# rasmusbarr/nudge

Hardware: AMD Instinct MI355X
Metric: simulation steps/s (contacts solved/s alongside), 1M-box drop scene (higher is better)
Workload: dtype f32

## Files before the change

### nudge_amd/csrc/nh_solve.hip

```cpp
#include "nh_internal.h"
int nh_asleep_remember(nh_context* ctx);
#include <type_traits>
#include <atomic>
#include <string.h>
#include "nh_solver.h"
#include "nh_narrowphase.h"

#define NH_NONE 0xFFFFFFFFu
#define NH_CLS_NONE 0u
#define NH_CLS_STATIC4 1u
#define NH_CLS_STATIC8 2u
#define NH_CLS_STATICN 3u
#define NH_CLS_GENERAL 4u
#define NH_CLS_PENDING 0xFFu
#define NH_CLS_STATIC4_LATE 5u
#define NH_CLS_STATIC8_LATE 6u
#define NH_UNSET 0xFFFFFFFFu

__device__ __forceinline__ bool tag_less(uint64_t ta, uint32_t fa, uint64_t tb, uint32_t fb) { return ta < tb || (ta == tb && fa < fb); }

__global__ __launch_bounds__(256) void k_gravity(const nh_DevState* __restrict__ st, const uint32_t* __restrict__ active, nh_BodyMomentum* __restrict__ momentum,
                                                 float gx_dt, float gy_dt, float gz_dt, float damping) {
	uint32_t n = st->active;
	for (uint32_t k = blockIdx.x * blockDim.x + threadIdx.x; k < n; k += gridDim.x * blockDim.x) {
// ... 858 lines not shown
		uint32_t nf[M], of[M];
		uint32_t sl[M], jm[M];
#pragma unroll
		for (int k = 0; k < M; ++k) { nf[k] = 0u; of[k] = 0u; sl[k] = (uint32_t)k; jm[k] = 0xFFFFFFFFu; }
		if (STILL) {
			still_has = br != NH_BODY_REC_NONE;
			still_rec = still_has ? (br & ~NH_BODY_REC_IS_A) : 0u;
			const uint32_t n_bb = min(cv.st->pairs, sv.pair_cap);
			still_base = still_rec < n_bb ? 4u * still_rec : 4u * n_bb + (still_rec - n_bb);
			const uint32_t bp = still_has ? bpos : 0u;
			st_cnt = sv.cnt_sorted[bp]; st_start = sv.start_sorted[bp]; st_oc = sv.sc_count[still_rec];
			if (PAIR) {
				const uint2 kp = still_rec < n_bb ? av.kept[still_rec] : av.kept[av.kept_cap - 1u - (still_rec - n_bb)];
				const uint64_t pk = av.rec_key[still_rec];
				s_pk[wave][0][lane] = kp.x; s_pk[wave][1][lane] = kp.y; s_pk[wave][2][lane] = (uint32_t)pk; s_pk[wave][3][lane] = (uint32_t)(pk >> 32);
			}
#pragma unroll
			for (int k = 0; k < M; ++k) { nf[k] = sv.raw_feature[still_base + k]; of[k] = sv.sc_feat[still_base + k]; }
			s_first[wave][lane] = still_has ? still_base : 0xFFFFFFFFu;
		} else {
		if (CONTIG) cnt = sp.y & 15u;
		else if (mine) { b = off[x]; cnt = off[x + 1] - b; }
#pragma unroll
		for (int q = 0; q < M; ++q) {
			if (CONTIG) cid[q] = (uint32_t)q < cnt ? sp.x + ((sp.y >> (4 + 3 * q)) & 7u) : 0xFFFFFFFFu;
			else cid[q] = (uint32_t)q < cnt ? adj[b + q] : 0xFFFFFFFFu;
			first = min(first, cid[q]);
		}
		}
		if (!STILL) {
#pragma unroll
			for (int q = 0; q < M; ++q) scid[lane * M + q] = cid[q];
			s_hint[wave][lane] = h; s_first[wave][lane] = first;
		}
		const bool ghost_lane = AHEAD && fs.ghost_first != 0u && x >= fs.ghost_first;
		if (AHEAD) { if (!mine || ghost_lane) col = 0xFFFFFFFFu; s_col[wave][lane] = col; }
		__builtin_amdgcn_wave_barrier();
		uint32_t sc[M], sflags[M];
		float4 sc0[M], sc1[M], sw[M];
		uint64_t stag[M], sctag[M];
		uint32_t sfeat[M], scfeat[M], sguess[M];
#pragma unroll
		for (int k = 0; k < M; ++k) {
			const uint32_t e = 64u * k + lane, j = e / M;
			if (STILL) { const uint32_t bj = s_first[wave][j]; sc[k] = bj != 0xFFFFFFFFu ? bj + (e - j * M) : 0xFFFFFFFFu; }
			else sc[k] = scid[e];
			const uint32_t c = sc[k] != 0xFFFFFFFFu ? sc[k] : 0u;
			sc0[k] = reinterpret_cast<const float4*>(contacts + c)[0];
			sc1[k] = reinterpret_cast<const float4*>(contacts + c)[1];
			sflags[k] = (!CONTIG && bodies[c].a == wave_x0 + j) ? 2u : 0u;
			if (STILL) {
				sw[k] = *reinterpret_cast<const float4*>(cv.cdata + c);
			} else if (FUSED) {
				const uint32_t hj = s_hint[wave][j];
				sguess[k] = hj != NH_HINT_NONE ? hj + (sc[k] - s_first[wave][j]) : sc[k];
				const uint32_t g = sguess[k] < m ? sguess[k] : 0u;
				stag[k] = cv.tags[c]; sfeat[k] = cv.features[c];
				sctag[k] = cv.ctags[g]; scfeat[k] = cv.cfeatures[g];
				sw[k] = *reinterpret_cast<const float4*>(cv.cdata + g);
			} else {
				sw[k] = states[c];
			}
		}
		float4 m0 = make_float4(0, 0, 0, 0), m1 = m0, pr = m0, t0 = m0, t1 = make_float4(0, 0, 0, 1);
		uint32_t idle_early = 0;
		if (mine) {
			m0 = reinterpret_cast<const float4*>(momentum + x)[0]; m1 = reinterpret_cast<const float4*>(momentum + x)[1];
			pr = *reinterpret_cast<const float4*>(props + x);
			t0 = reinterpret_cast<const float4*>(xf + x)[0]; t1 = reinterpret_cast<const float4*>(xf + x)[1];
			if (CONTIG && (fs.bits & 2u)) idle_early = (STILL && (fs.bits & 4u)) ? idle0 : fs.idle[x];
			if (CONTIG && (fs.bits & 1u)) {
				float vel[3] = { m0.x, m0.y, m0.z }, ang[3] = { m1.x, m1.y, m1.z };
				nh_gravity_damping(vel, ang, fs.gx_dt, fs.gy_dt, fs.gz_dt, fs.damping);
				m0.x = vel[0]; m0.y = vel[1]; m0.z = vel[2]; m1.x = ang[0]; m1.y = ang[1]; m1.z = ang[2];
			}
		}
#pragma unroll
		for (int k = 0; k < M; ++k) {
			const uint32_t e = 64u * k + lane;
			nh_ob_slot o;
			o.c0 = make_float4(0, 0, 0, 0); o.c1 = o.c0; o.w = o.c0;
			if (sc[k] != 0xFFFFFFFFu) {
				uint32_t flags = sflags[k];
				o.c0 = sc0[k]; o.c1 = sc1[k];
				if (STILL) {
					o.w = make_float4(sw[k].x, sw[k].y, sw[k].z, __uint_as_float(flags));
				} else if (FUSED) {
					const bool hit = sguess[k] < m && sctag[k] == stag[k] && scfeat[k] == sfeat[k];
					if (!hit) flags |= 1u;
					o.w = hit ? make_float4(sw[k].x, sw[k].y, sw[k].z, __uint_as_float(flags)) : make_float4(0.0f, 0.0f, 0.0f, __uint_as_float(flags));
				} else {
					o.w = make_float4(sw[k].x, sw[k].y, sw[k].z, __uint_as_float(flags));
				}
			}
			slot[e] = o;
		}
		if (STILL) {
			uint32_t oc = 0;
			if (still_has) {
				cnt = min(st_cnt, 4u); oc = min(st_oc, 4u);
				uint32_t start = st_start;
				int shift = 0;
				for (uint32_t k = 0; k < n_delta; ++k) shift += (uint32_t)s_delta[k].x < bpos ? s_delta[k].y : 0;
				if (shift) { start += (uint32_t)shift; sv.start_sorted[bpos] = start; }
				st_start = start;
			}
			uint32_t ci[M], key[M];
#pragma unroll
			for (int k = 0; k < M; ++k) {
				uint32_t r = 0;
#pragma unroll
				for (int j = 0; j < M; ++j) r += ((uint32_t)j < cnt && (uint32_t)k < cnt && (nf[j] < nf[k] || (nf[j] == nf[k] && j < k))) ? 1u : 0u;
				const bool on = (uint32_t)k < cnt;
				ci[k] = on ? st_start + r : 0xFFFFFFFFu;
				key[k] = on ? slot_key_of(ci[k], nullptr) : 0xFFFFFFFFu;
				sl[k] = (uint32_t)k;
			}
#pragma unroll
			for (int q = 1; q < M; ++q) {
#pragma unroll
				for (int j = q; j > 0; --j) {
					const bool sw2 = (key[j] < key[j - 1]) || (key[j] == key[j - 1] && ci[j] < ci[j - 1]);
					const uint32_t tc = sw2 ? ci[j - 1] : ci[j], tk = sw2 ? key[j - 1] : key[j], ts = sw2 ? sl[j - 1] : sl[j];
					ci[j - 1] = sw2 ? ci[j] : ci[j - 1]; key[j - 1] = sw2 ? key[j] : key[j - 1]; sl[j - 1] = sw2 ? sl[j] : sl[j - 1];
					ci[j] = tc; key[j] = tk; sl[j] = ts;
				}
			}
#pragma unroll
			for (int q = 0; q < M; ++q) {
				const bool on = (uint32_t)q < cnt;
				uint32_t f = 0, wj = 0xFFFFFFFFu;
#pragma unroll
				for (int k = 0; k < M; ++k) if (sl[q] == (uint32_t)k) f = nf[k];
#pragma unroll
				for (int j = M - 1; j >= 0; --j) if ((uint32_t)j < oc && of[j] == f) wj = (uint32_t)j;
				jm[q] = on ? wj : 0xFFFFFFFFu;
				cid[q] = on ? still_base + sl[q] : 0xFFFFFFFFu;
				scid[lane * M + q] = cid[q];
			}
			if (still_has) {
#pragma unroll
				for (int k = 0; k < M; ++k) if ((uint32_t)k < cnt) sv.sc_feat[still_base + k] = nf[k];
				sv.sc_count[still_rec] = cnt;
			}
		}
		__builtin_amdgcn_wave_barrier();
		nh_vel v = { m0.x, m0.y, m0.z, pr.w, m1.x, m1.y, m1.z, m1.w };
		const nh_quat qx = { t1.x, t1.y, t1.z, t1.w };
		const nh_inertia IX = nh_world_inertia(qx, pr.x, pr.y, pr.z);
		const nh_f3 posx = nh_make3(t0.x, t0.y, t0.z);
		nh_row1 r[M];
		nh_state s[M];
		bool is_a[M];
#pragma unroll
		for (int q = 0; q < M; ++q) {
			is_a[q] = false;
			if ((uint32_t)q < cnt) {
				const nh_ob_slot o = slot[lane * M + (STILL ? sl[q] : (uint32_t)q)];
				const uint32_t flags = STILL ? 0u : __float_as_uint(o.w.w);
				is_a[q] = STILL ? (br & NH_BODY_REC_IS_A) != 0 : (CONTIG ? ((sp.y >> 28) & 1u) != 0 : (flags & 2u) != 0);
				nh_contact_in ci = { o.c0.x, o.c0.y, o.c0.z, o.c0.w, o.c1.x, o.c1.y, o.c1.z, o.c1.w };
				nh_build_row1(ci, posx, IX, v.mass_inverse, is_a[q], r[q]);
				if (FUSED) {
					float wx = o.w.x, wy = o.w.y, wz = o.w.z;
					if (STILL) {
						const float4 wv = slot[lane * M + (jm[q] != 0xFFFFFFFFu ? jm[q] : 0u)].w;
						const bool hit = jm[q] != 0xFFFFFFFFu;
						wx = hit ? wv.x : 0.0f; wy = hit ? wv.y : 0.0f; wz = hit ? wv.z : 0.0f;
					}
					if (!STILL && (flags & 1u)) {
						const float4 found = cache_search(cv.ctags, cv.cfeatures, cv.cdata, m, h != NH_HINT_NONE ? h + (cid[q] - first) : cid[q], cv.tags[cid[q]], cv.features[cid[q]]);
						wx = found.x; wy = found.y; wz = found.z;
					}
					nh_warm_start1(r[q], wx, wy, wz, v, is_a[q], s[q]);
				} else {
					s[q].normal = o.w.x; s[q].friction_x = o.w.y; s[q].friction_y = o.w.z;
				}
			}
		}
		if (FUSED && !STILL && mine) hint[x] = first;
		nh_xform pp_x = nh_xform();
		float4 pp_min = make_float4(0, 0, 0, 0), pp_max = pp_min, pp_shape = pp_min;
		uint32_t pp_tag = 0, pp_own_tag = 0, pp_partner = 0xFFFFFFFFu, pp_bits = 0;
		if (PAIR && CONTIG && (fs.bits & 2u) && mine && still_has && s_col[wave][lane] != 0xFFFFFFFFu) {
			const uint32_t ah_col = s_col[wave][lane];
			const uint32_t kx = s_pk[wave][0][lane], ky = s_pk[wave][1][lane];
			const uint32_t index_mask = av.gen ? NH_GEN_INDEX : 0xFFFFFFFFu;
			const uint32_t ca = kx & index_mask, cb = ky & index_mask;
			pp_partner = ca == ah_col ? cb : ca;
			pp_bits = 1u | ((ca != ah_col && cb != ah_col) ? 4u : 0u);
			if (av.gen && cv.st->moved_count != 0u && !((uint32_t)(av.gen[ca] & 0x7Fu) == (kx >> NH_GEN_SHIFT) && (uint32_t)(av.gen[cb] & 0x7Fu) == (ky >> NH_GEN_SHIFT))) pp_bits |= 2u;
			pp_x = av.xf[pp_partner]; pp_min = av.aabb_min[pp_partner]; pp_max = av.aabb_max[pp_partner];
			if (pp_partner < av.nbox) pp_shape = *reinterpret_cast<const float4*>(av.box_data + pp_partner);
			else pp_shape.x = av.sph_data[pp_partner - av.nbox].radius;
			pp_tag = av.ctag[pp_partner]; pp_own_tag = av.ctag[ah_col];
		}
		float4* const s_ah = reinterpret_cast<float4*>(slot);
		float ah_rad = 0.0f;
		if (AHEAD) {
			__builtin_amdgcn_wave_barrier();
			const uint32_t c0 = s_col[wave][lane];
			const uint32_t cc = c0 != 0xFFFFFFFFu ? c0 : 0u;
			const bool is_box = cc < av.nbox;
			const float4* lp = reinterpret_cast<const float4*>(is_box ? av.box_xf + cc : av.sph_xf + (cc - av.nbox));
			const float4* sp4 = is_box ? reinterpret_cast<const float4*>(av.box_data + cc) : lp;
			if (!is_box) ah_rad = av.sph_data[cc - av.nbox].radius;
			nh_glds16(lp, &s_ah[lane]); nh_glds16(lp + 1, &s_ah[64u + lane]);
			nh_glds16(av.fat_box + 2u * (size_t)cc, &s_ah[128u + lane]); nh_glds16(av.fat_box + 2u * (size_t)cc + 1u, &s_ah[192u + lane]);
			nh_glds16(sp4, &s_ah[256u + lane]);
		}
		if (CONTIG && __builtin_amdgcn_ballot_w64(mine && (STILL ? (still_has && (br & NH_BODY_REC_IS_A) != 0) : ((sp.y >> 28) & 1u) != 0)) == 0) {
			for (uint32_t it = 0; it < iterations; ++it) {
#pragma unroll
				for (int q = 0; q < M; ++q)
					if ((uint32_t)q < cnt) nh_apply_one1(r[q], s[q], v, false);
			}
		} else {
			for (uint32_t it = 0; it < iterations; ++it) {
#pragma unroll
				for (int q = 0; q < M; ++q)
					if ((uint32_t)q < cnt) nh_apply_one1(r[q], s[q], v, is_a[q]);
			}
		}
		float4 a0 = make_float4(0, 0, 0, 0), a1 = a0;
		uint32_t idle_in = 0;
		const bool advance_here = CONTIG && (fs.bits & 2u) && mine;
		float4 ah_l0 = make_float4(0, 0, 0, 0), ah_l1 = ah_l0, ah_fmn = ah_l0, ah_fmx = ah_l0, ah_sz = ah_l0;
		uint32_t ah_col = 0xFFFFFFFFu;
		if (AHEAD) {
			ah_col = s_col[wave][lane];
			asm volatile("s_waitcnt vmcnt(0)" ::: "memory");
			ah_l0 = s_ah[lane]; ah_l1 = s_ah[64u + lane]; ah_fmn = s_ah[128u + lane]; ah_fmx = s_ah[192u + lane]; ah_sz = s_ah[256u + lane];
		}
		if (advance_here) { a0 = t0; a1 = t1; idle_in = idle_early; }
		__builtin_amdgcn_wave_barrier();
#pragma unroll
		for (int q = 0; q < M; ++q) {
			if ((uint32_t)q < cnt) {
				float ox, oy, oz;
				nh_export_impulse1(r[q], s[q], ox, oy, oz);
				slot[lane * M + q].c0 = make_float4(s[q].normal, s[q].friction_x, s[q].friction_y, 0.0f);
				slot[lane * M + q].c1 = make_float4(ox, oy, oz, 0.0f);
			}
		}
		__builtin_amdgcn_wave_barrier();
#pragma unroll
		for (int k = 0; k < M; ++k) {
			const uint32_t e = 64u * k + lane;
			const uint32_t c = scid[e];
			if (c != 0xFFFFFFFFu) {
				if (keep_states) states[c] = slot[e].c0;
				*reinterpret_cast<float4*>(out_impulses + c) = slot[e].c1;
			}
		}
		if (mine) {
			reinterpret_cast<float4*>(momentum + x)[0] = make_float4(v.vx, v.vy, v.vz, v.mass_inverse);
			reinterpret_cast<float4*>(momentum + x)[1] = make_float4(v.wx, v.wy, v.wz, v.w_unused);
		}
		uint32_t nmin[3] = { 0xffffffffu, 0xffffffffu, 0xffffffffu }, nmax[3] = { 0u, 0u, 0u }, ntop = 0u;
		bool nfail = false;
		int pp_count = 0;
		float pair_scale = 0.0f;
		if (PAIR) {
			__builtin_amdgcn_wave_barrier();
#pragma unroll
			for (int k = 0; k < M; ++k) scid[lane * M + k] = 0xFFFFFFFFu;
			const nh_DevState* const sp = cv.st;
			const nh_f3 smin = nh_make3(nh_float_unflip(sp->still_smin[sv.parity][0]), nh_float_unflip(sp->still_smin[sv.parity][1]), nh_float_unflip(sp->still_smin[sv.parity][2]));
			const nh_f3 smax = nh_make3(nh_float_unflip(sp->still_smax[sv.parity][0]), nh_float_unflip(sp->still_smax[sv.parity][1]), nh_float_unflip(sp->still_smax[sv.parity][2]));
			pair_scale = nh_morton_scale(smin, smax);
			if (sp->pair_unowned > av.unowned_cap) nfail = true;
		}
		if (advance_here) {
			float pos[3] = { a0.x, a0.y, a0.z }, rot[4] = { a1.x, a1.y, a1.z, a1.w };
			const float vel[3] = { v.vx, v.vy, v.vz }, ang[3] = { v.wx, v.wy, v.wz };
			const uint8_t idle_out = nh_advance_body(pos, rot, vel, ang, (uint8_t)idle_in, fs.time_step);
			fs.idle[x] = idle_out;
			reinterpret_cast<float4*>(xf + x)[0] = make_float4(pos[0], pos[1], pos[2], a0.w);
			reinterpret_cast<float4*>(xf + x)[1] = make_float4(rot[0], rot[1], rot[2], rot[3]);
			if (AHEAD && !ghost_lane) {
				ntop = idle_out; nfail = idle_out == 0xffu;
				const uint32_t c = ah_col;
				if (c != 0xFFFFFFFFu) {
					const bool is_box = c < av.nbox;
					const float4 l0 = ah_l0, l1 = ah_l1, fmn = ah_fmn, fmx = ah_fmx;
					float4 sz = ah_sz;
					if (!is_box) sz.x = ah_rad;
					const nh_quat bq = { rot[0], rot[1], rot[2], rot[3] };
					const nh_quat lq = { l1.x, l1.y, l1.z, l1.w };
					const nh_f3 p = nh_rotate(bq, nh_make3(l0.x, l0.y, l0.z)) + nh_make3(pos[0], pos[1], pos[2]);
					const nh_quat q = nh_qmul(bq, lq);
					float sx, sy, sz2;
					if (is_box) {
						const nh_m33 m = nh_matrix(q);
						const nh_f3 c0 = m.c0 * sz.x, c1 = m.c1 * sz.y, c2 = m.c2 * sz.z;
						sx = fabsf(c0.x) + fabsf(c1.x) + fabsf(c2.x);
						sy = fabsf(c0.y) + fabsf(c1.y) + fabsf(c2.y);
						sz2 = fabsf(c0.z) + fabsf(c1.z) + fabsf(c2.z);
					} else {
						sx = sy = sz2 = sz.x;
					}
					const float mnx = p.x - sx, mny = p.y - sy, mnz = p.z - sz2, mxx = p.x + sx, mxy = p.y + sy, mxz = p.z + sz2;
					float4* const wx = reinterpret_cast<float4*>(av.xf) + 2u * (size_t)c;
					wx[0] = make_float4(p.x, p.y, p.z, l0.w);
					wx[1] = make_float4(q.x, q.y, q.z, q.s);
					av.aabb_min[c] = make_float4(mnx, mny, mnz, l0.w);
					av.aabb_max[c] = make_float4(mxx, mxy, mxz, __uint_as_float(0u));
					nfail |= !(mnx >= fmn.x && mny >= fmn.y && mnz >= fmn.z && mxx <= fmx.x && mxy <= fmx.y && mxz <= fmx.z);
					nmin[0] = nmax[0] = nh_float_flip(mnx); nmin[1] = nmax[1] = nh_float_flip(mny); nmin[2] = nmax[2] = nh_float_flip(mnz);
					if (PAIR && (pp_bits & 1u)) {
						const float4 omin = make_float4(mnx, mny, mnz, l0.w), omax = make_float4(mxx, mxy, mxz, 0.0f);
						nh_xform OX; OX.px = p.x; OX.py = p.y; OX.pz = p.z; OX.body = __float_as_uint(l0.w); OX.qx = q.x; OX.qy = q.y; OX.qz = q.z; OX.qs = q.s;
						const bool hit = nh_aabb_overlap(omin, omax, pp_min, pp_max) && __float_as_uint(pp_min.w) != OX.body && !(pp_bits & 2u);
						const float ddx = mnx - pp_min.x, ddy = mny - pp_min.y, ddz = mnz - pp_min.z;
						const float far = 2.0f;
						const bool partner_first = ddx >= 0.0f && ddy >= 0.0f && ddz >= 0.0f && fmaxf(fmaxf(ddx, ddy), ddz) * pair_scale >= far;
						const bool own_first = ddx <= 0.0f && ddy <= 0.0f && ddz <= 0.0f && fmaxf(fmaxf(-ddx, -ddy), -ddz) * pair_scale >= far;
						bool pfail = (pp_bits & 4u) != 0u || (hit && !partner_first && !own_first) || __float_as_uint(pp_min.w) != 0u;
						if (pfail) atomicAdd(&const_cast<nh_DevState*>(cv.st)->pair_diag[(hit && !partner_first && !own_first) ? 0 : 1], 1u);
						uint64_t key = ~0ull;
						uint32_t body_a = 0, body_b = 0;
						nh_bb_result bb;
						bb.kind = 0; bb.mask = 0;
						nh_contact_out single;
						single.px = single.py = single.pz = single.penetration = single.nx = single.ny = single.nz = 0.0f; single.friction = 0.5f; single.feature = 0u;
						if (hit && !pfail) {
							const bool a_is_own = partner_first;
							const nh_xform A = a_is_own ? OX : pp_x, B = a_is_own ? pp_x : OX;
							const uint32_t ta = a_is_own ? pp_own_tag : pp_tag, tb = a_is_own ? pp_tag : pp_own_tag;
							const bool own_sph = !is_box, par_sph = pp_partner >= av.nbox;
							const bool a_sph = a_is_own ? own_sph : par_sph, b_sph = a_is_own ? par_sph : own_sph;
							const float own_size[3] = { sz.x, sz.y, sz.z }, par_size[3] = { pp_shape.x, pp_shape.y, pp_shape.z };
							const float ra = a_is_own ? sz.x : pp_shape.x, rb = a_is_own ? pp_shape.x : sz.x;
							if (!a_sph && !b_sph) {
								nh_box_box_eval(A, B, a_is_own ? own_size : par_size, a_is_own ? par_size : own_size, ta, tb, bb);
								pp_count = nh_bb_count(bb);
								key = (uint64_t)(bb.swapped ? tb : ta) | ((uint64_t)(bb.swapped ? ta : tb) << 32);
								body_a = bb.swapped ? B.body : A.body; body_b = bb.swapped ? A.body : B.body;
							} else if (a_sph && b_sph) {
								pp_count = nh_sphere_sphere(rb, ra, B, A, &single);
								key = (uint64_t)tb | ((uint64_t)ta << 32);
								body_a = B.body; body_b = A.body;
							} else {
								const nh_xform BX = a_sph ? B : A, SP = a_sph ? A : B;
								const bool box_is_own = a_sph ? !a_is_own : a_is_own;
								pp_count = nh_box_sphere(box_is_own ? own_size : par_size, a_sph ? ra : rb, BX, SP, &single);
								key = (uint64_t)(a_sph ? tb : ta) | ((uint64_t)(a_sph ? ta : tb) << 32);
								body_a = BX.body; body_b = SP.body;
							}
						}
						{
							const uint64_t was_key = (uint64_t)s_pk[wave][2][lane] | ((uint64_t)s_pk[wave][3][lane] << 32);
							const bool vanished = !hit;
							const bool same_key = was_key == key || vanished;
							bool ok = same_key && pp_count <= 4;
							if (ok && pp_count) ok = (body_a == 0u) != (body_b == 0u);
							if (!ok) { pfail = true; pp_count = 0; bb.kind = 0; atomicAdd(&const_cast<nh_DevState*>(cv.st)->pair_diag[1], 1u); }
						}
						nfail |= pfail;
						if (pp_count) {
							nh_ob_slot* const stage = slot + lane * M;
							if (bb.kind == 2) {
								int k = 0;
#pragma unroll
								for (int index = 0; index < 16; ++index) {
									if (((bb.mask >> index) & 1u) && k < pp_count && k < M) {
										nh_contact_out o;
										nh_bb_contact(bb, index, bb.fx[index], bb.fy[index], bb.fz[index], bb.penetration[index], bb.tags[index], o);
										stage[k].c0 = make_float4(o.px, o.py, o.pz, o.penetration); stage[k].c1 = make_float4(o.nx, o.ny, o.nz, o.friction); stage[k].w.x = __uint_as_float(o.feature);
										scid[lane * M + k] = still_base + (uint32_t)k;
										++k;
									}
								}
							} else {
								const nh_contact_out o = bb.kind == 1 ? bb.edge : single;
// ... 1955 lines not shown
```

### nudge_amd/csrc/nh_solver.h

```cpp
#ifndef NH_SOLVER_H
#define NH_SOLVER_H

#include "nh_math.h"

#if defined(NH_SOLVER_EXACT_DIV)
NH_HD float nh_recip_s(float x) { return nh_recip(x); }
NH_HD float nh_rsqrt_s(float x) { return nh_rsqrt(x); }
#else
NH_HD float nh_recip_s(float x) { return nh_recip_guarded(x); }
NH_HD float nh_rsqrt_s(float x) { return nh_rsqrt_guarded_z(x); }
#endif

struct nh_inertia { float xx, yy, zz, xy, xz, yz; };

NH_HD nh_inertia nh_world_inertia(nh_quat q, float ix, float iy, float iz) {
	nh_m33 m = nh_matrix(q);
	nh_inertia t;
	t.xx = ix * m.c0.x * m.c0.x + iy * m.c1.x * m.c1.x + iz * m.c2.x * m.c2.x;
	t.yy = ix * m.c0.y * m.c0.y + iy * m.c1.y * m.c1.y + iz * m.c2.y * m.c2.y;
	t.zz = ix * m.c0.z * m.c0.z + iy * m.c1.z * m.c1.z + iz * m.c2.z * m.c2.z;
	t.xy = ix * m.c0.x * m.c0.y + iy * m.c1.x * m.c1.y + iz * m.c2.x * m.c2.y;
	t.xz = ix * m.c0.x * m.c0.z + iy * m.c1.x * m.c1.z + iz * m.c2.x * m.c2.z;
	t.yz = ix * m.c0.y * m.c0.z + iy * m.c1.y * m.c1.z + iz * m.c2.y * m.c2.z;
	return t;
}

struct nh_row {
	float pa_z, pa_x, pa_y;
	float pb_z, pb_x, pb_y;
	float n_x, u_x, v_x;
	float n_y, u_y, v_y;
	float n_z, u_z, v_z;
	float bias, friction, normal_velocity_to_normal_impulse;
	float friction_coefficient_x, friction_coefficient_y, friction_coefficient_z;
	float na_x, na_y, na_z;
	float nb_x, nb_y, nb_z;
	float ua_x, ua_y, ua_z;
	float va_x, va_y, va_z;
	float ub_x, ub_y, ub_z;
	float vb_x, vb_y, vb_z;
	float pad;
};

struct nh_state { float normal, friction_x, friction_y; };

struct nh_vel { float vx, vy, vz, mass_inverse, wx, wy, wz, w_unused; };

struct nh_contact_in { float px, py, pz, penetration, nx, ny, nz, friction; };

#define NH_ALLOWED_PENETRATION 1e-3f
#define NH_BIAS_FACTOR 2.0f

NH_HD void nh_build_row(const nh_contact_in& c, nh_f3 apos, nh_f3 bpos, const nh_inertia& A, const nh_inertia& B,
                        float a_mass_inverse, float b_mass_inverse, nh_row& r) {
	float nx = c.nx, ny = c.ny, nz = c.nz;
	float pa_x = c.px - apos.x, pa_y = c.py - apos.y, pa_z = c.pz - apos.z;
	float pb_x = c.px - bpos.x, pb_y = c.py - bpos.y, pb_z = c.pz - bpos.z;

	float na_xt = pa_y * nz - pa_z * ny, na_yt = pa_z * nx - pa_x * nz, na_zt = pa_x * ny - pa_y * nx;
	float na_x = A.xx * na_xt + A.xy * na_yt + A.xz * na_zt;
	float na_y = A.xy * na_xt + A.yy * na_yt + A.yz * na_zt;
	float na_z = A.xz * na_xt + A.yz * na_yt + A.zz * na_zt;

	float nb_xt = pb_y * nz - pb_z * ny, nb_yt = pb_z * nx - pb_x * nz, nb_zt = pb_x * ny - pb_y * nx;
	float nb_x = B.xx * nb_xt + B.xy * nb_yt + B.xz * nb_zt;
	float nb_y = B.xy * nb_xt + B.yy * nb_yt + B.yz * nb_zt;
	float nb_z = B.xz * nb_xt + B.yz * nb_yt + B.zz * nb_zt;

	na_xt = na_y * pa_z - na_z * pa_y; na_yt = na_z * pa_x - na_x * pa_z; na_zt = na_x * pa_y - na_y * pa_x;
	nb_xt = nb_y * pb_z - nb_z * pb_y; nb_yt = nb_z * pb_x - nb_x * pb_z; nb_zt = nb_x * pb_y - nb_y * pb_x;

	float rx = na_xt + nb_xt, ry = na_yt + nb_yt, rz = na_zt + nb_zt;
	float r_dot_n = rx * nx + ry * ny + rz * nz;

	float mass_inverse = a_mass_inverse + b_mass_inverse;
	float nvtni = mass_inverse + r_dot_n;
	bool nonzero = (nvtni < 0.0f) || (nvtni > 0.0f);
	nvtni = nonzero ? nh_neg(nh_recip_s(nvtni)) : 0.0f;

	float bias = (-NH_BIAS_FACTOR) * nh_max(c.penetration - NH_ALLOWED_PENETRATION, 0.0f) * nvtni;

	float s = nh_abs(nx);
	float u_x = nz * s;
	float u_y = u_x - nz;
	float u_z = nh_madd(nx - ny, s, ny);
	u_x = nh_neg(u_x);
	{
		float f = nh_rsqrt_s(u_x * u_x + u_y * u_y + u_z * u_z);
		u_x *= f; u_y *= f; u_z *= f;
	}
	float v_x = u_y * nz - u_z * ny, v_y = u_z * nx - u_x * nz, v_z = u_x * ny - u_y * nx;

	float ua_x = pa_y * u_z - pa_z * u_y, ua_y = pa_z * u_x - pa_x * u_z, ua_z = pa_x * u_y - pa_y * u_x;
	float va_x = pa_y * v_z - pa_z * v_y, va_y = pa_z * v_x - pa_x * v_z, va_z = pa_x * v_y - pa_y * v_x;
	float ub_x = pb_y * u_z - pb_z * u_y, ub_y = pb_z * u_x - pb_x * u_z, ub_z = pb_x * u_y - pb_y * u_x;
	float vb_x = pb_y * v_z - pb_z * v_y, vb_y = pb_z * v_x - pb_x * v_z, vb_z = pb_x * v_y - pb_y * v_x;

	float a_duu = A.xx * ua_x * ua_x + A.yy * ua_y * ua_y + A.zz * ua_z * ua_z;
	float a_dvv = A.xx * va_x * va_x + A.yy * va_y * va_y + A.zz * va_z * va_z;
	float a_duv = A.xx * ua_x * va_x + A.yy * ua_y * va_y + A.zz * ua_z * va_z;
	float a_suu = A.xy * ua_x * ua_y + A.xz * ua_x * ua_z + A.yz * ua_y * ua_z;
	float a_svv = A.xy * va_x * va_y + A.xz * va_x * va_z + A.yz * va_y * va_z;
	float a_suv = A.xy * (ua_x * va_y + ua_y * va_x) + A.xz * (ua_x * va_z + ua_z * va_x) + A.yz * (ua_y * va_z + ua_z * va_y);

	float b_duu = B.xx * ub_x * ub_x + B.yy * ub_y * ub_y + B.zz * ub_z * ub_z;
	float b_dvv = B.xx * vb_x * vb_x + B.yy * vb_y * vb_y + B.zz * vb_z * vb_z;
	float b_duv = B.xx * ub_x * vb_x + B.yy * ub_y * vb_y + B.zz * ub_z * vb_z;
	float b_suu = B.xy * ub_x * ub_y + B.xz * ub_x * ub_z + B.yz * ub_y * ub_z;
	float b_svv = B.xy * vb_x * vb_y + B.xz * vb_x * vb_z + B.yz * vb_y * vb_z;
	float b_suv = B.xy * (ub_x * vb_y + ub_y * vb_x) + B.xz * (ub_x * vb_z + ub_z * vb_x) + B.yz * (ub_y * vb_z + ub_z * vb_y);

	float friction_x = mass_inverse + a_duu + a_suu + a_suu + b_duu + b_suu + b_suu;
	float friction_y = mass_inverse + a_dvv + a_svv + a_svv + b_dvv + b_svv + b_svv;
	float friction_z = a_duv + a_duv + a_suv + a_suv + b_duv + b_duv + b_suv + b_suv;

	float ua_xt = A.xx * ua_x + A.xy * ua_y + A.xz * ua_z;
	float ua_yt = A.xy * ua_x + A.yy * ua_y + A.yz * ua_z;
	float ua_zt = A.xz * ua_x + A.yz * ua_y + A.zz * ua_z;
	float va_xt = A.xx * va_x + A.xy * va_y + A.xz * va_z;
	float va_yt = A.xy * va_x + A.yy * va_y + A.yz * va_z;
	float va_zt = A.xz * va_x + A.yz * va_y + A.zz * va_z;
	float ub_xt = B.xx * ub_x + B.xy * ub_y + B.xz * ub_z;
	float ub_yt = B.xy * ub_x + B.yy * ub_y + B.yz * ub_z;
	float ub_zt = B.xz * ub_x + B.yz * ub_y + B.zz * ub_z;
	float vb_xt = B.xx * vb_x + B.xy * vb_y + B.xz * vb_z;
	float vb_yt = B.xy * vb_x + B.yy * vb_y + B.yz * vb_z;
	float vb_zt = B.xz * vb_x + B.yz * vb_y + B.zz * vb_z;

	r.pa_x = pa_x; r.pa_y = pa_y; r.pa_z = pa_z;
	r.pb_x = pb_x; r.pb_y = pb_y; r.pb_z = pb_z;
	r.n_x = nx; r.n_y = ny; r.n_z = nz;
	r.u_x = u_x; r.u_y = u_y; r.u_z = u_z;
	r.v_x = v_x; r.v_y = v_y; r.v_z = v_z;
	r.bias = bias; r.friction = c.friction; r.normal_velocity_to_normal_impulse = nvtni;
	r.friction_coefficient_x = friction_x; r.friction_coefficient_y = friction_y; r.friction_coefficient_z = friction_z;
	r.ua_x = nh_neg(ua_xt); r.ua_y = nh_neg(ua_yt); r.ua_z = nh_neg(ua_zt);
	r.va_x = nh_neg(va_xt); r.va_y = nh_neg(va_yt); r.va_z = nh_neg(va_zt);
	r.na_x = nh_neg(na_x); r.na_y = nh_neg(na_y); r.na_z = nh_neg(na_z);
	r.ub_x = ub_xt; r.ub_y = ub_yt; r.ub_z = ub_zt;
	r.vb_x = vb_xt; r.vb_y = vb_yt; r.vb_z = vb_zt;
	r.nb_x = nb_x; r.nb_y = nb_y; r.nb_z = nb_z;
	r.pad = 0.0f;
}

NH_HD void nh_warm_start(const nh_row& r, float cix, float ciy, float ciz, nh_vel& a, nh_vel& b, nh_state& st) {
	float normal_impulse = nh_max(r.n_x * cix + r.n_y * ciy + r.n_z * ciz, 0.0f);
	float max_friction_impulse = normal_impulse * r.friction;
	float fx = r.u_x * cix + r.u_y * ciy + r.u_z * ciz;
	float fy = r.v_x * cix + r.v_y * ciy + r.v_z * ciz;
	float scale = fx * fx + fy * fy;
	scale = nh_rsqrt_s(scale);
	scale = scale * max_friction_impulse;
	scale = nh_min(1.0f, scale);
	fx = fx * scale;
	fy = fy * scale;

	float lx = fx * r.u_x + fy * r.v_x + r.n_x * normal_impulse;
	float ly = fx * r.u_y + fy * r.v_y + r.n_y * normal_impulse;
	float lz = fx * r.u_z + fy * r.v_z + r.n_z * normal_impulse;

	float aax = fx * r.ua_x + fy * r.va_x + normal_impulse * r.na_x;
	float aay = fx * r.ua_y + fy * r.va_y + normal_impulse * r.na_y;
	float aaz = fx * r.ua_z + fy * r.va_z + normal_impulse * r.na_z;
// ... 73 lines not shown
	a.wx = nh_madd(r.na_x, normal_impulse, a.wx);
	a.wy = nh_madd(r.na_y, normal_impulse, a.wy);
	a.wz = nh_madd(r.na_z, normal_impulse, a.wz);

	float old_friction_impulse_x = st.friction_x, old_friction_impulse_y = st.friction_y;

	friction_factor = nh_min(1e+6f, friction_factor);

	float friction_impulse_x = t_x * friction_factor;
	float friction_impulse_y = t_y * friction_factor;

	friction_impulse_x = old_friction_impulse_x - friction_impulse_x;
	friction_impulse_y = old_friction_impulse_y - friction_impulse_y;

	float friction_clamp_scale = friction_impulse_x * friction_impulse_x + friction_impulse_y * friction_impulse_y;
	friction_clamp_scale = nh_rsqrt_s(friction_clamp_scale);

	b.wx = nh_madd(r.nb_x, normal_impulse, b.wx);
	b.wy = nh_madd(r.nb_y, normal_impulse, b.wy);
	b.wz = nh_madd(r.nb_z, normal_impulse, b.wz);

	friction_clamp_scale = friction_clamp_scale * max_friction_impulse;
	friction_clamp_scale = nh_min(1.0f, friction_clamp_scale);

	friction_impulse_x = friction_impulse_x * friction_clamp_scale;
	friction_impulse_y = friction_impulse_y * friction_clamp_scale;

	st.friction_x = friction_impulse_x;
	st.friction_y = friction_impulse_y;

	friction_impulse_x -= old_friction_impulse_x;
	friction_impulse_y -= old_friction_impulse_y;

	linear_impulse_x = nh_madd(r.u_x, friction_impulse_x, linear_impulse_x);
	linear_impulse_y = nh_madd(r.u_y, friction_impulse_x, linear_impulse_y);
	linear_impulse_z = nh_madd(r.u_z, friction_impulse_x, linear_impulse_z);

	linear_impulse_x = nh_madd(r.v_x, friction_impulse_y, linear_impulse_x);
	linear_impulse_y = nh_madd(r.v_y, friction_impulse_y, linear_impulse_y);
	linear_impulse_z = nh_madd(r.v_z, friction_impulse_y, linear_impulse_z);

	float a_mass_inverse_neg = nh_neg(a.mass_inverse);

	a.vx = nh_madd(linear_impulse_x, a_mass_inverse_neg, a.vx);
	a.vy = nh_madd(linear_impulse_y, a_mass_inverse_neg, a.vy);
	a.vz = nh_madd(linear_impulse_z, a_mass_inverse_neg, a.vz);

	a.wx = nh_madd(r.ua_x, friction_impulse_x, a.wx);
	a.wy = nh_madd(r.ua_y, friction_impulse_x, a.wy);
	a.wz = nh_madd(r.ua_z, friction_impulse_x, a.wz);

	a.wx = nh_madd(r.va_x, friction_impulse_y, a.wx);
	a.wy = nh_madd(r.va_y, friction_impulse_y, a.wy);
	a.wz = nh_madd(r.va_z, friction_impulse_y, a.wz);

	a.w_unused = 0.0f;

	b.vx = nh_madd(linear_impulse_x, b.mass_inverse, b.vx);
	b.vy = nh_madd(linear_impulse_y, b.mass_inverse, b.vy);
	b.vz = nh_madd(linear_impulse_z, b.mass_inverse, b.vz);

	b.wx = nh_madd(r.ub_x, friction_impulse_x, b.wx);
	b.wy = nh_madd(r.ub_y, friction_impulse_x, b.wy);
	b.wz = nh_madd(r.ub_z, friction_impulse_x, b.wz);

	b.wx = nh_madd(r.vb_x, friction_impulse_y, b.wx);
	b.wy = nh_madd(r.vb_y, friction_impulse_y, b.wy);
	b.wz = nh_madd(r.vb_z, friction_impulse_y, b.wz);

	b.w_unused = 0.0f;
}


struct nh_row1 {
	float p_z, p_x, p_y;
	float n_x, u_x, v_x;
	float n_y, u_y, v_y;
	float n_z, u_z, v_z;
	float bias, friction, normal_velocity_to_normal_impulse;
	float friction_coefficient_x, friction_coefficient_y, friction_coefficient_z;
	float nd_x, nd_y, nd_z;
	float ud_x, ud_y, ud_z;
	float vd_x, vd_y, vd_z;
};

NH_HD void nh_build_row1(const nh_contact_in& c, nh_f3 dpos, const nh_inertia& D, float d_mass_inverse, bool d_is_a, nh_row1& r) {
	float nx = c.nx, ny = c.ny, nz = c.nz;
	float p_x = c.px - dpos.x, p_y = c.py - dpos.y, p_z = c.pz - dpos.z;

	float n_xt = p_y * nz - p_z * ny, n_yt = p_z * nx - p_x * nz, n_zt = p_x * ny - p_y * nx;
	float nd_x = D.xx * n_xt + D.xy * n_yt + D.xz * n_zt;
	float nd_y = D.xy * n_xt + D.yy * n_yt + D.yz * n_zt;
	float nd_z = D.xz * n_xt + D.yz * n_yt + D.zz * n_zt;

	float rx = nd_y * p_z - nd_z * p_y, ry = nd_z * p_x - nd_x * p_z, rz = nd_x * p_y - nd_y * p_x;
	float r_dot_n = rx * nx + ry * ny + rz * nz;

	float mass_inverse = d_mass_inverse;
	float nvtni = mass_inverse + r_dot_n;
	bool nonzero = (nvtni < 0.0f) || (nvtni > 0.0f);
	nvtni = nonzero ? nh_neg(nh_recip_s(nvtni)) : 0.0f;

	float bias = (-NH_BIAS_FACTOR) * nh_max(c.penetration - NH_ALLOWED_PENETRATION, 0.0f) * nvtni;

	float s = nh_abs(nx);
	float u_x = nz * s;
	float u_y = u_x - nz;
	float u_z = nh_madd(nx - ny, s, ny);
	u_x = nh_neg(u_x);
	{
		float f = nh_rsqrt_s(u_x * u_x + u_y * u_y + u_z * u_z);
		u_x *= f; u_y *= f; u_z *= f;
	}
	float v_x = u_y * nz - u_z * ny, v_y = u_z * nx - u_x * nz, v_z = u_x * ny - u_y * nx;

	float ud_x = p_y * u_z - p_z * u_y, ud_y = p_z * u_x - p_x * u_z, ud_z = p_x * u_y - p_y * u_x;
	float vd_x = p_y * v_z - p_z * v_y, vd_y = p_z * v_x - p_x * v_z, vd_z = p_x * v_y - p_y * v_x;

	float duu = D.xx * ud_x * ud_x + D.yy * ud_y * ud_y + D.zz * ud_z * ud_z;
	float dvv = D.xx * vd_x * vd_x + D.yy * vd_y * vd_y + D.zz * vd_z * vd_z;
	float duv = D.xx * ud_x * vd_x + D.yy * ud_y * vd_y + D.zz * ud_z * vd_z;
	float suu = D.xy * ud_x * ud_y + D.xz * ud_x * ud_z + D.yz * ud_y * ud_z;
	float svv = D.xy * vd_x * vd_y + D.xz * vd_x * vd_z + D.yz * vd_y * vd_z;
	float suv = D.xy * (ud_x * vd_y + ud_y * vd_x) + D.xz * (ud_x * vd_z + ud_z * vd_x) + D.yz * (ud_y * vd_z + ud_z * vd_y);

	float friction_x = mass_inverse + duu + suu + suu;
	float friction_y = mass_inverse + dvv + svv + svv;
	float friction_z = duv + duv + suv + suv;

	float ud_xt = D.xx * ud_x + D.xy * ud_y + D.xz * ud_z;
	float ud_yt = D.xy * ud_x + D.yy * ud_y + D.yz * ud_z;
	float ud_zt = D.xz * ud_x + D.yz * ud_y + D.zz * ud_z;
	float vd_xt = D.xx * vd_x + D.xy * vd_y + D.xz * vd_z;
	float vd_yt = D.xy * vd_x + D.yy * vd_y + D.yz * vd_z;
	float vd_zt = D.xz * vd_x + D.yz * vd_y + D.zz * vd_z;

	r.p_x = p_x; r.p_y = p_y; r.p_z = p_z;
	r.n_x = nx; r.n_y = ny; r.n_z = nz;
	r.u_x = u_x; r.u_y = u_y; r.u_z = u_z;
	r.v_x = v_x; r.v_y = v_y; r.v_z = v_z;
	r.bias = bias; r.friction = c.friction; r.normal_velocity_to_normal_impulse = nvtni;
	r.friction_coefficient_x = friction_x; r.friction_coefficient_y = friction_y; r.friction_coefficient_z = friction_z;
	if (d_is_a) {
		r.nd_x = nh_neg(nd_x); r.nd_y = nh_neg(nd_y); r.nd_z = nh_neg(nd_z);
		r.ud_x = nh_neg(ud_xt); r.ud_y = nh_neg(ud_yt); r.ud_z = nh_neg(ud_zt);
		r.vd_x = nh_neg(vd_xt); r.vd_y = nh_neg(vd_yt); r.vd_z = nh_neg(vd_zt);
	} else {
		r.nd_x = nd_x; r.nd_y = nd_y; r.nd_z = nd_z;
		r.ud_x = ud_xt; r.ud_y = ud_yt; r.ud_z = ud_zt;
		r.vd_x = vd_xt; r.vd_y = vd_yt; r.vd_z = vd_zt;
	}
}

NH_HD void nh_warm_start1(const nh_row1& r, float cix, float ciy, float ciz, nh_vel& d, bool d_is_a, nh_state& st) {
	float normal_impulse = nh_max(r.n_x * cix + r.n_y * ciy + r.n_z * ciz, 0.0f);
	float max_friction_impulse = normal_impulse * r.friction;
	float fx = r.u_x * cix + r.u_y * ciy + r.u_z * ciz;
	float fy = r.v_x * cix + r.v_y * ciy + r.v_z * ciz;
	float scale = fx * fx + fy * fy;
	scale = nh_rsqrt_s(scale);
	scale = scale * max_friction_impulse;
	scale = nh_min(1.0f, scale);
	fx = fx * scale;
	fy = fy * scale;

	float lx = fx * r.u_x + fy * r.v_x + r.n_x * normal_impulse;
	float ly = fx * r.u_y + fy * r.v_y + r.n_y * normal_impulse;
	float lz = fx * r.u_z + fy * r.v_z + r.n_z * normal_impulse;

	float ax = fx * r.ud_x + fy * r.vd_x + normal_impulse * r.nd_x;
	float ay = fx * r.ud_y + fy * r.vd_y + normal_impulse * r.nd_y;
	float az = fx * r.ud_z + fy * r.vd_z + normal_impulse * r.nd_z;

	if (d_is_a) { d.vx -= lx * d.mass_inverse; d.vy -= ly * d.mass_inverse; d.vz -= lz * d.mass_inverse; }
	else        { d.vx += lx * d.mass_inverse; d.vy += ly * d.mass_inverse; d.vz += lz * d.mass_inverse; }
	d.wx += ax; d.wy += ay; d.wz += az;

	st.normal = normal_impulse; st.friction_x = fx; st.friction_y = fy;
}

NH_HD void nh_apply_one1(const nh_row1& r, nh_state& st, nh_vel& d, bool d_is_a) {
	float l_x = nh_madd(d.wy, r.p_z, d.vx);
	float l_y = nh_madd(d.wz, r.p_x, d.vy);
	float l_z = nh_madd(d.wx, r.p_y, d.vz);
	float c_x = nh_madd(d.wz, r.p_y, 0.0f);
	float c_y = nh_madd(d.wx, r.p_z, 0.0f);
	float c_z = nh_madd(d.wy, r.p_x, 0.0f);
	float v_x = d_is_a ? (c_x - l_x) : (l_x - c_x);
	float v_y = d_is_a ? (c_y - l_y) : (l_y - c_y);
	float v_z = d_is_a ? (c_z - l_z) : (l_z - c_z);

	float t_z = r.n_x * v_x;
	float t_x = v_x * r.u_x;
	float t_y = v_x * r.v_x;

	float normal_bias = r.bias;
	float old_normal_impulse = st.normal;
	float normal_factor = r.normal_velocity_to_normal_impulse;

	t_z = nh_madd(r.n_y, v_y, t_z);
	t_x = nh_madd(v_y, r.u_y, t_x);
	t_y = nh_madd(v_y, r.v_y, t_y);

	normal_bias = normal_bias + old_normal_impulse;

	t_z = nh_madd(r.n_z, v_z, t_z);
	t_x = nh_madd(v_z, r.u_z, t_x);
	t_y = nh_madd(v_z, r.v_z, t_y);

	float normal_impulse = nh_madd(normal_factor, t_z, normal_bias);

	float t_xx = t_x * t_x, t_yy = t_y * t_y, t_xy = t_x * t_y;
	float tl2 = t_xx + t_yy;

	normal_impulse = nh_max(normal_impulse, 0.0f);

	t_x *= tl2;
	t_y *= tl2;

	st.normal = normal_impulse;

	float max_friction_impulse = normal_impulse * r.friction;
	normal_impulse = normal_impulse - old_normal_impulse;

	float friction_factor = t_xx * r.friction_coefficient_x;
	float linear_impulse_x = r.n_x * normal_impulse;
	friction_factor = nh_madd(t_yy, r.friction_coefficient_y, friction_factor);
	float linear_impulse_y = r.n_y * normal_impulse;
	friction_factor = nh_madd(t_xy, r.friction_coefficient_z, friction_factor);
	float linear_impulse_z = r.n_z * normal_impulse;

	friction_factor = nh_recip_s(friction_factor);

	d.wx = nh_madd(r.nd_x, normal_impulse, d.wx);
	d.wy = nh_madd(r.nd_y, normal_impulse, d.wy);
	d.wz = nh_madd(r.nd_z, normal_impulse, d.wz);

	float old_friction_impulse_x = st.friction_x, old_friction_impulse_y = st.friction_y;

	friction_factor = nh_min(1e+6f, friction_factor);

	float friction_impulse_x = t_x * friction_factor;
	float friction_impulse_y = t_y * friction_factor;

	friction_impulse_x = old_friction_impulse_x - friction_impulse_x;
	friction_impulse_y = old_friction_impulse_y - friction_impulse_y;

	float friction_clamp_scale = friction_impulse_x * friction_impulse_x + friction_impulse_y * friction_impulse_y;
	friction_clamp_scale = nh_rsqrt_s(friction_clamp_scale);

	friction_clamp_scale = friction_clamp_scale * max_friction_impulse;
	friction_clamp_scale = nh_min(1.0f, friction_clamp_scale);

	friction_impulse_x = friction_impulse_x * friction_clamp_scale;
	friction_impulse_y = friction_impulse_y * friction_clamp_scale;

	st.friction_x = friction_impulse_x;
	st.friction_y = friction_impulse_y;

	friction_impulse_x -= old_friction_impulse_x;
	friction_impulse_y -= old_friction_impulse_y;

	linear_impulse_x = nh_madd(r.u_x, friction_impulse_x, linear_impulse_x);
	linear_impulse_y = nh_madd(r.u_y, friction_impulse_x, linear_impulse_y);
	linear_impulse_z = nh_madd(r.u_z, friction_impulse_x, linear_impulse_z);

	linear_impulse_x = nh_madd(r.v_x, friction_impulse_y, linear_impulse_x);
	linear_impulse_y = nh_madd(r.v_y, friction_impulse_y, linear_impulse_y);
	linear_impulse_z = nh_madd(r.v_z, friction_impulse_y, linear_impulse_z);

	float signed_mass_inverse = d_is_a ? nh_neg(d.mass_inverse) : d.mass_inverse;

	d.vx = nh_madd(linear_impulse_x, signed_mass_inverse, d.vx);
	d.vy = nh_madd(linear_impulse_y, signed_mass_inverse, d.vy);
	d.vz = nh_madd(linear_impulse_z, signed_mass_inverse, d.vz);

	d.wx = nh_madd(r.ud_x, friction_impulse_x, d.wx);
	d.wy = nh_madd(r.ud_y, friction_impulse_x, d.wy);
	d.wz = nh_madd(r.ud_z, friction_impulse_x, d.wz);

	d.wx = nh_madd(r.vd_x, friction_impulse_y, d.wx);
	d.wy = nh_madd(r.vd_y, friction_impulse_y, d.wy);
	d.wz = nh_madd(r.vd_z, friction_impulse_y, d.wz);

	d.w_unused = 0.0f;
}

NH_HD void nh_export_impulse1(const nh_row1& r, const nh_state& st, float& ix, float& iy, float& iz) {
	ix = st.normal * r.n_x + st.friction_x * r.u_x + st.friction_y * r.v_x;
	iy = st.normal * r.n_y + st.friction_x * r.u_y + st.friction_y * r.v_y;
	iz = st.normal * r.n_z + st.friction_x * r.u_z + st.friction_y * r.v_z;
}

struct nh_rowr {
	float n_x, n_y, n_z, bias;
	float alpha, beta, friction, normal_velocity_to_normal_impulse;
	float friction_coefficient, c_a, c_b, pad;
};

NH_HD void nh_rowr_derive(float alpha, float beta, float a_mass_inverse, float b_mass_inverse, float k_a, float k_b, float& friction_coefficient, float& c_a, float& c_b) {
	float mass_inverse = a_mass_inverse + b_mass_inverse;
	friction_coefficient = mass_inverse + k_a * alpha * alpha + k_b * beta * beta;
	c_a = k_a * alpha; c_b = k_b * beta;
}

NH_HD void nh_tangents(float nx, float ny, float nz, nh_f3& u, nh_f3& v) {
	float s = nh_abs(nx);
	float u_x = nz * s;
	float u_y = u_x - nz;
	float u_z = nh_madd(nx - ny, s, ny);
	u_x = nh_neg(u_x);
	float f = nh_rsqrt_s(u_x * u_x + u_y * u_y + u_z * u_z);
	u_x *= f; u_y *= f; u_z *= f;
	u = nh_make3(u_x, u_y, u_z);
	v = nh_make3(u_y * nz - u_z * ny, u_z * nx - u_x * nz, u_x * ny - u_y * nx);
}

NH_HD bool nh_side_is_radial(float px, float py, float pz, float nx, float ny, float nz, float ix, float iy, float iz, bool inert) {
	if (inert) return true;
	if (!(nh_asuint(ix) == nh_asuint(iy) && nh_asuint(iy) == nh_asuint(iz))) return false;
	float cx = py * nz - pz * ny, cy = pz * nx - px * nz, cz = px * ny - py * nx;
	return cx * cx + cy * cy + cz * cz <= 1e-6f * (px * px + py * py + pz * pz);
}

NH_HD void nh_build_rowr(const nh_contact_in& c, nh_f3 apos, nh_f3 bpos, float k_a, float k_b, float a_mass_inverse, float b_mass_inverse,
                         bool a_inert, bool b_inert, nh_rowr& r) {
	float alpha = a_inert ? 0.0f : (c.px - apos.x) * c.nx + (c.py - apos.y) * c.ny + (c.pz - apos.z) * c.nz;
	float beta = b_inert ? 0.0f : (c.px - bpos.x) * c.nx + (c.py - bpos.y) * c.ny + (c.pz - bpos.z) * c.nz;
	float mass_inverse = a_mass_inverse + b_mass_inverse;
	bool nonzero = (mass_inverse < 0.0f) || (mass_inverse > 0.0f);
	float nvtni = nonzero ? nh_neg(nh_recip_s(mass_inverse)) : 0.0f;
	r.n_x = c.nx; r.n_y = c.ny; r.n_z = c.nz;
	r.bias = (-NH_BIAS_FACTOR) * nh_max(c.penetration - NH_ALLOWED_PENETRATION, 0.0f) * nvtni;
	r.alpha = alpha; r.beta = beta;
	r.normal_velocity_to_normal_impulse = nvtni;
	nh_rowr_derive(alpha, beta, a_mass_inverse, b_mass_inverse, k_a, k_b, r.friction_coefficient, r.c_a, r.c_b);
	r.friction = c.friction; r.pad = 0.0f;
}

NH_HD void nh_warm_start_r(const nh_rowr& r, float cix, float ciy, float ciz, nh_vel& a, nh_vel& b, nh_state& st) {
	nh_f3 u, v;
	nh_tangents(r.n_x, r.n_y, r.n_z, u, v);
	float normal_impulse = nh_max(r.n_x * cix + r.n_y * ciy + r.n_z * ciz, 0.0f);
	float max_friction_impulse = normal_impulse * r.friction;
	float fx = u.x * cix + u.y * ciy + u.z * ciz;
	float fy = v.x * cix + v.y * ciy + v.z * ciz;
	float scale = fx * fx + fy * fy;
	scale = nh_rsqrt_s(scale);
	scale = scale * max_friction_impulse;
	scale = nh_min(1.0f, scale);
	fx = fx * scale;
	fy = fy * scale;
	float lx = fx * u.x + fy * v.x + r.n_x * normal_impulse;
	float ly = fx * u.y + fy * v.y + r.n_y * normal_impulse;
	float lz = fx * u.z + fy * v.z + r.n_z * normal_impulse;
	float wx = fx * v.x - fy * u.x, wy = fx * v.y - fy * u.y, wz = fx * v.z - fy * u.z;
	a.vx -= lx * a.mass_inverse; a.vy -= ly * a.mass_inverse; a.vz -= lz * a.mass_inverse;
	a.wx += r.c_a * wx; a.wy += r.c_a * wy; a.wz += r.c_a * wz;
	b.vx += lx * b.mass_inverse; b.vy += ly * b.mass_inverse; b.vz += lz * b.mass_inverse;
	b.wx -= r.c_b * wx; b.wy -= r.c_b * wy; b.wz -= r.c_b * wz;
	st.normal = normal_impulse; st.friction_x = fx; st.friction_y = fy;
}

NH_HD void nh_apply_radial(const nh_rowr& r, nh_state& st, nh_vel& a, nh_vel& b) {
	nh_f3 u, v;
	nh_tangents(r.n_x, r.n_y, r.n_z, u, v);
	float dwx = r.beta * b.wx - r.alpha * a.wx, dwy = r.beta * b.wy - r.alpha * a.wy, dwz = r.beta * b.wz - r.alpha * a.wz;
	float v_x = (b.vx - a.vx) + (dwy * r.n_z - dwz * r.n_y);
	float v_y = (b.vy - a.vy) + (dwz * r.n_x - dwx * r.n_z);
	float v_z = (b.vz - a.vz) + (dwx * r.n_y - dwy * r.n_x);

	float t_z = nh_madd(r.n_z, v_z, nh_madd(r.n_y, v_y, r.n_x * v_x));
	float t_x = nh_madd(v_z, u.z, nh_madd(v_y, u.y, v_x * u.x));
	float t_y = nh_madd(v_z, v.z, nh_madd(v_y, v.y, v_x * v.x));

	float old_normal_impulse = st.normal;
	float normal_impulse = nh_madd(r.normal_velocity_to_normal_impulse, t_z, r.bias + old_normal_impulse);
	float t_xx = t_x * t_x, t_yy = t_y * t_y;
	float tl2 = t_xx + t_yy;
	normal_impulse = nh_max(normal_impulse, 0.0f);
	t_x *= tl2;
	t_y *= tl2;
	st.normal = normal_impulse;
	float max_friction_impulse = normal_impulse * r.friction;
	normal_impulse = normal_impulse - old_normal_impulse;

	float friction_factor = nh_madd(t_yy, r.friction_coefficient, t_xx * r.friction_coefficient);
	friction_factor = nh_recip_s(friction_factor);
	friction_factor = nh_min(1e+6f, friction_factor);

	float old_fx = st.friction_x, old_fy = st.friction_y;
	float fx = old_fx - t_x * friction_factor;
	float fy = old_fy - t_y * friction_factor;
	float clamp = nh_rsqrt_s(fx * fx + fy * fy);
	clamp = clamp * max_friction_impulse;
	clamp = nh_min(1.0f, clamp);
	fx = fx * clamp;
	fy = fy * clamp;
	st.friction_x = fx;
	st.friction_y = fy;
	fx -= old_fx;
	fy -= old_fy;
// ... 76 lines not shown
```

Before: 3698.

## Use fast unguarded recip/rsqrt in solver with wave-level fallback replay

Replaces the guarded reciprocal and rsqrt in the per-body contact solver sweeps with fast versions. Each call records a wave-wide ballot flag when a result is out of range or the input is near zero. If any lane in the wave is flagged, the velocity and warm-start state are restored from saved copies and all sweeps rerun with exact division. This removes guard instructions from the hot inner loop. In exchange it keeps extra registers for the saved state and pays a full replay whenever a wave hits a bad value.

Result: faster. 3797 (median of 6 runs) (+2.7%).

```diff
diff --git a/nudge_amd/csrc/nh_solve.hip b/nudge_amd/csrc/nh_solve.hip
--- a/nudge_amd/csrc/nh_solve.hip
+++ b/nudge_amd/csrc/nh_solve.hip
@@ -1034,9 +1034,13 @@
 		nh_row1 r[M];
 		nh_state s[M];
 		bool is_a[M];
+		nh_div_deferred dd;
+		const nh_vel v0 = v;
+		nh_state w0[M];
 #pragma unroll
 		for (int q = 0; q < M; ++q) {
 			is_a[q] = false;
+			w0[q].normal = 0.0f; w0[q].friction_x = 0.0f; w0[q].friction_y = 0.0f;
 			if ((uint32_t)q < cnt) {
 				const nh_ob_slot o = slot[lane * M + (STILL ? sl[q] : (uint32_t)q)];
 				const uint32_t flags = STILL ? 0u : __float_as_uint(o.w.w);
@@ -1054,9 +1058,11 @@
 						const float4 found = cache_search(cv.ctags, cv.cfeatures, cv.cdata, m, h != NH_HINT_NONE ? h + (cid[q] - first) : cid[q], cv.tags[cid[q]], cv.features[cid[q]]);
 						wx = found.x; wy = found.y; wz = found.z;
 					}
-					nh_warm_start1(r[q], wx, wy, wz, v, is_a[q], s[q]);
+					w0[q].normal = wx; w0[q].friction_x = wy; w0[q].friction_y = wz;
+					nh_warm_start1(r[q], wx, wy, wz, v, is_a[q], s[q], dd);
 				} else {
-					s[q].normal = o.w.x; s[q].friction_x = o.w.y; s[q].friction_y = o.w.z;
+					w0[q].normal = o.w.x; w0[q].friction_x = o.w.y; w0[q].friction_y = o.w.z;
+					s[q] = w0[q];
 				}
 			}
 		}
@@ -1091,18 +1097,34 @@
 			nh_glds16(av.fat_box + 2u * (size_t)cc, &s_ah[128u + lane]); nh_glds16(av.fat_box + 2u * (size_t)cc + 1u, &s_ah[192u + lane]);
 			nh_glds16(sp4, &s_ah[256u + lane]);
 		}
-		if (CONTIG && __builtin_amdgcn_ballot_w64(mine && (STILL ? (still_has && (br & NH_BODY_REC_IS_A) != 0) : ((sp.y >> 28) & 1u) != 0)) == 0) {
-			for (uint32_t it = 0; it < iterations; ++it) {
-#pragma unroll
-				for (int q = 0; q < M; ++q)
-					if ((uint32_t)q < cnt) nh_apply_one1(r[q], s[q], v, false);
-			}
-		} else {
-			for (uint32_t it = 0; it < iterations; ++it) {
-#pragma unroll
-				for (int q = 0; q < M; ++q)
-					if ((uint32_t)q < cnt) nh_apply_one1(r[q], s[q], v, is_a[q]);
-			}
+		const bool none_a = CONTIG && __builtin_amdgcn_ballot_w64(mine && (STILL ? (still_has && (br & NH_BODY_REC_IS_A) != 0) : ((sp.y >> 28) & 1u) != 0)) == 0;
+		auto sweeps = [&](auto& div) {
+			if (none_a) {
+				for (uint32_t it = 0; it < iterations; ++it) {
+#pragma unroll
+					for (int q = 0; q < M; ++q)
+						if ((uint32_t)q < cnt) nh_apply_one1(r[q], s[q], v, false, div);
+				}
+			} else {
+				for (uint32_t it = 0; it < iterations; ++it) {
+#pragma unroll
+					for (int q = 0; q < M; ++q)
+						if ((uint32_t)q < cnt) nh_apply_one1(r[q], s[q], v, is_a[q], div);
+				}
+			}
+		};
+		sweeps(dd);
+		if (__builtin_expect(dd.bad != 0ull, 0)) {
+			nh_div_exact ex;
+			v = v0;
+#pragma unroll
+			for (int q = 0; q < M; ++q) {
+				if ((uint32_t)q < cnt) {
+					if (FUSED) nh_warm_start1(r[q], w0[q].normal, w0[q].friction_x, w0[q].friction_y, v, is_a[q], s[q], ex);
+					else s[q] = w0[q];
+				}
+			}
+			sweeps(ex);
 		}
 		float4 a0 = make_float4(0, 0, 0, 0), a1 = a0;
 		uint32_t idle_in = 0;
diff --git a/nudge_amd/csrc/nh_solver.h b/nudge_amd/csrc/nh_solver.h
--- a/nudge_amd/csrc/nh_solver.h
+++ b/nudge_amd/csrc/nh_solver.h
@@ -9,6 +9,24 @@
 #else
 NH_HD float nh_recip_s(float x) { return nh_recip_guarded(x); }
 NH_HD float nh_rsqrt_s(float x) { return nh_rsqrt_guarded_z(x); }
+#endif
+
+struct nh_div_exact {
+	NH_HD float recip(float x) { return nh_recip(x); }
+	NH_HD float rsqrt(float x) { return nh_rsqrt(x); }
+};
+#if defined(__HIP_DEVICE_COMPILE__) && !defined(NH_SOLVER_EXACT_DIV)
+struct nh_div_deferred {
+	uint64_t bad = 0;
+	__device__ __forceinline__ float recip(float x) { float r = nh_recip_fast_z(x); bad |= __builtin_amdgcn_ballot_w64(nh_recip_fast_z_bad(r)); return r; }
+	__device__ __forceinline__ float rsqrt(float x) {
+		float r = nh_rsqrt_fast_z(x);
+		bad |= __builtin_amdgcn_ballot_w64(nh_rsqrt_fast_z_bad(r)) | (__builtin_amdgcn_ballot_w64(nh_rsqrt_fast_z_small(x)) & ~__builtin_amdgcn_ballot_w64(x == 0.0f));
+		return r;
+	}
+};
+#else
+struct nh_div_deferred : nh_div_exact { uint64_t bad = 0; };
 #endif
 
 struct nh_inertia { float xx, yy, zz, xy, xz, yz; };
@@ -388,13 +406,14 @@
 	}
 }
 
-NH_HD void nh_warm_start1(const nh_row1& r, float cix, float ciy, float ciz, nh_vel& d, bool d_is_a, nh_state& st) {
+template <class DIV = nh_div_exact>
+NH_HD void nh_warm_start1(const nh_row1& r, float cix, float ciy, float ciz, nh_vel& d, bool d_is_a, nh_state& st, DIV&& div = DIV()) {
 	float normal_impulse = nh_max(r.n_x * cix + r.n_y * ciy + r.n_z * ciz, 0.0f);
 	float max_friction_impulse = normal_impulse * r.friction;
 	float fx = r.u_x * cix + r.u_y * ciy + r.u_z * ciz;
 	float fy = r.v_x * cix + r.v_y * ciy + r.v_z * ciz;
 	float scale = fx * fx + fy * fy;
-	scale = nh_rsqrt_s(scale);
+	scale = div.rsqrt(scale);
 	scale = scale * max_friction_impulse;
 	scale = nh_min(1.0f, scale);
 	fx = fx * scale;
@@ -415,7 +434,8 @@
 	st.normal = normal_impulse; st.friction_x = fx; st.friction_y = fy;
 }
 
-NH_HD void nh_apply_one1(const nh_row1& r, nh_state& st, nh_vel& d, bool d_is_a) {
+template <class DIV = nh_div_exact>
+NH_HD void nh_apply_one1(const nh_row1& r, nh_state& st, nh_vel& d, bool d_is_a, DIV&& div = DIV()) {
 	float l_x = nh_madd(d.wy, r.p_z, d.vx);
 	float l_y = nh_madd(d.wz, r.p_x, d.vy);
 	float l_z = nh_madd(d.wx, r.p_y, d.vz);
@@ -466,7 +486,7 @@
 	friction_factor = nh_madd(t_xy, r.friction_coefficient_z, friction_factor);
 	float linear_impulse_z = r.n_z * normal_impulse;
 
-	friction_factor = nh_recip_s(friction_factor);
+	friction_factor = div.recip(friction_factor);
 
 	d.wx = nh_madd(r.nd_x, normal_impulse, d.wx);
 	d.wy = nh_madd(r.nd_y, normal_impulse, d.wy);
@@ -483,7 +503,7 @@
 	friction_impulse_y = old_friction_impulse_y - friction_impulse_y;
 
 	float friction_clamp_scale = friction_impulse_x * friction_impulse_x + friction_impulse_y * friction_impulse_y;
-	friction_clamp_scale = nh_rsqrt_s(friction_clamp_scale);
+	friction_clamp_scale = div.rsqrt(friction_clamp_scale);
 
 	friction_clamp_scale = friction_clamp_scale * max_friction_impulse;
 	friction_clamp_scale = nh_min(1.0f, friction_clamp_scale);
```
